# LaurenYTaylor/jsrl-CORL

Hardware: NVIDIA B200
Metric: iql_gradient_steps_per_sec_summed_over_seeds (higher is better)
Workload: dtype tf32

## Files before the change

include/iql_b200.h:

```cpp
#ifndef IQL_B200_H
#define IQL_B200_H

#include <stddef.h>
#include <stdint.h>

#ifdef __cplusplus
extern "C" {
#endif

#define IQL_OK 0
#define IQL_ERR_INVALID 1
#define IQL_ERR_CUDA 2
#define IQL_ERR_STATE 3
#define IQL_ERR_SHAPE 4

#define IQL_MATH_FP32_SIMT 0
#define IQL_MATH_TF32_TCGEN05 1

#define IQL_SAMPLE_PHILOX 0
#define IQL_SAMPLE_INDICES 1
#define IQL_SAMPLE_PRELOADED 2

#define IQL_NET_Q1 0
#define IQL_NET_Q2 1
// ... 144 lines not shown
                         float* host_out, float* host_std, void* stream, void* caller_stream);
int iql_get_act_steps(iql_engine* e, uint64_t* host_out);
int iql_set_act_steps(iql_engine* e, const uint64_t* host_in);
int iql_replay_insert_members_host(iql_engine* e, const float* host_states, const float* host_actions,
                                   const float* host_rewards, const float* host_next_states, const float* host_dones,
                                   const int64_t* host_pointers, void* stream, void* caller_stream);
int iql_selftest_umma_gemm(int32_t mode, int32_t M, int32_t N, int32_t K, const float* A, int32_t lda,
                           const float* B, int32_t ldb, float* C, int32_t ldc, void* scratch,
                           size_t scratch_bytes, void* stream);
int iql_profile_step(iql_engine* e, int32_t reps, int32_t max_slots, int32_t* n_slots, float* avg_ms,
                     double* flops, double* bytes, char* labels, void* stream);
int64_t iql_last_launch_count(const iql_engine* e);
int iql_debug_fused_trace(long long* out, int32_t max_words);
int iql_debug_step_trace(iql_engine* e, int32_t reset, unsigned long long* out, int32_t max_words, void* stream);
int iql_debug_chain_trace(long long* out, int32_t max_words);

#ifdef __cplusplus
}
#endif
#endif
```

jsrl_corl_b200/_lib.py:

```python
from __future__ import annotations

import ctypes as C
import os

_HERE = os.path.dirname(os.path.abspath(__file__))
LIB_PATH = os.path.join(_HERE, "libiql_b200.so")
if os.environ.get("IQL_B200_DEBUG") and os.environ.get("IQL_B200_LIB"):
    LIB_PATH = os.environ["IQL_B200_LIB"]

IQL_OK, IQL_ERR_INVALID, IQL_ERR_CUDA, IQL_ERR_STATE, IQL_ERR_SHAPE = 0, 1, 2, 3, 4
MATH_FP32_SIMT, MATH_TF32_TCGEN05 = 0, 1
SAMPLE_PHILOX, SAMPLE_INDICES, SAMPLE_PRELOADED = 0, 1, 2
NET_Q1, NET_Q2, NET_V, NET_ACTOR = 0, 1, 2, 3
KIND_WEIGHT, KIND_BIAS, KIND_LOG_STD = 0, 1, 2
OPT_STEP_PATH, OPT_KEEP_GRADS = 1, 2
INFO_TENSOR_CORE_PATH, INFO_FUSED_FORWARD, INFO_CHAINED_BACKWARD, INFO_CHAINED_BACKWARD_GRADS = 1, 2, 3, 4
STEP_PATHS = {"auto": 0, "phases": 1, "chain": 2, "chain_grads": 4}
ACT_SKIP, ACT_LEARNER, ACT_LEARNER_DIST, ACT_GUIDE, ACT_LEARNER_DROPOUT, ACT_LEARNER_DIST_DROPOUT = 0, 1, 2, 3, 4, 5
ACT_SOURCES = {"skip": ACT_SKIP, "learner": ACT_LEARNER, "learner_dist": ACT_LEARNER_DIST, "guide": ACT_GUIDE,
               "learner_dropout": ACT_LEARNER_DROPOUT, "learner_dist_dropout": ACT_LEARNER_DIST_DROPOUT}


class Config(C.Structure):
    _fields_ = [
# ... 82 lines not shown
    "iql_load_batch": (C.c_int, [_P, C.c_int32, _P, _P, _P, _P, _P, _P]),
    "iql_train_steps": (C.c_int, [_P, C.c_int32, C.c_int32, _P, _P, _P, _P, _P]),
    "iql_train_host_step": (C.c_int, [_P, _P, _P, _P, _P]),
    "iql_host_step_wait": (C.c_int, [_P, _P, _P]),
    "iql_act": (C.c_int, [_P, C.c_int32, _P, C.c_int64, C.c_float, _P, _P]),
    "iql_act_host": (C.c_int, [_P, C.c_int32, _P, C.c_float, _P, _P, _P]),
    "iql_act_host_gaussian": (C.c_int, [_P, C.c_int32, _P, _P, _P, _P, _P]),
    "iql_bind_guide": (C.c_int, [_P, _P]),
    "iql_act_host_members": (C.c_int, [_P, _P, _P, C.c_float, _P, _P, _P, _P]),
    "iql_get_act_steps": (C.c_int, [_P, _P]),
    "iql_set_act_steps": (C.c_int, [_P, _P]),
    "iql_replay_insert_members_host": (C.c_int, [_P, _P, _P, _P, _P, _P, _P, _P, _P]),
    "iql_last_launch_count": (C.c_int64, [_P]),
    "iql_debug_fused_trace": (C.c_int, [_P, C.c_int32]),
    "iql_debug_chain_trace": (C.c_int, [_P, C.c_int32]),
    "iql_debug_step_trace": (C.c_int, [_P, C.c_int32, _P, C.c_int32, _P]),
    "iql_profile_step": (C.c_int, [_P, C.c_int32, C.c_int32, C.POINTER(C.c_int32), _P, _P, _P, _P, _P]),
    "iql_selftest_umma_gemm": (C.c_int, [C.c_int32, C.c_int32, C.c_int32, C.c_int32, _P, C.c_int32, _P, C.c_int32,
                                          _P, C.c_int32, _P, C.c_size_t, _P]),
}

_LIB = None


def lib() -> C.CDLL:
    global _LIB
    if _LIB is None:
        if not os.path.exists(LIB_PATH):
            raise RuntimeError(
                f"{LIB_PATH} is missing: the CUDA engine is the only compute path of jsrl_corl_b200 "
# ... 35 lines not shown
```

jsrl_corl_b200/csrc/common.cuh:

```cuda
#pragma once
#include <cuda_runtime.h>
#include <stdint.h>
#include <stdlib.h>
#include <string.h>

namespace iql {

#define IQL_PHILOX_M0 0xD2511F53u
#define IQL_PHILOX_M1 0xCD9E8D57u
#define IQL_PHILOX_W0 0x9E3779B9u
#define IQL_PHILOX_W1 0xBB67AE85u

#define IQL_STREAM_SAMPLE 0u
#define IQL_STREAM_DROPOUT_BASE 1u
#define IQL_STREAM_ACT_DROPOUT_BASE 0x80000000u

struct Philox4 {
  uint32_t x, y, z, w;
};

__host__ __device__ __forceinline__ void philox_mulhilo(uint32_t a, uint32_t b, uint32_t& hi, uint32_t& lo) {
  uint64_t p = (uint64_t)a * (uint64_t)b;
  hi = (uint32_t)(p >> 32);
  lo = (uint32_t)p;
// ... 48 lines not shown
  return (uint32_t)t;
}

__device__ __forceinline__ float round_tf32(float x) {
  return __uint_as_float((__float_as_uint(x) + 0x1000u) & 0xFFFFE000u);
}

static inline int64_t round_up(int64_t x, int64_t m) { return (x + m - 1) / m * m; }

static inline const char* dbg_getenv(const char* name) {
  static int on = -1;
  if (on < 0) on = getenv("IQL_B200_DEBUG") ? 1 : 0;
  return on ? getenv(name) : nullptr;
}

__device__ __forceinline__ void stamp_begin(unsigned long long* stamps, int slot) {
  if (stamps && threadIdx.x == 0) {
    unsigned long long t;
    asm volatile("mov.u64 %0, %%globaltimer;" : "=l"(t));
    atomicMin(stamps + 2 * slot, t);
  }
}
__device__ __forceinline__ void stamp_end(unsigned long long* stamps, int slot) {
  if (stamps && threadIdx.x == 0) {
    unsigned long long t;
    asm volatile("mov.u64 %0, %%globaltimer;" : "=l"(t));
    atomicMax(stamps + 2 * slot + 1, t);
  }
}

// ... 48 lines not shown
```

jsrl_corl_b200/csrc/engine.cu:

```cuda
#include <math.h>
#include <stdio.h>
#include <string.h>

#include <algorithm>
#include <atomic>
#include <chrono>
#include <map>
#include <tuple>
#include <string>
#include <type_traits>
#include <vector>

#include "common.cuh"
#include "engine.h"
#include "umma_gemm.h"

using namespace iql;

static thread_local std::string g_create_error;
static constexpr int CHAIN_GRADS_MIN_MEMBERS = 8;

struct StepTimer {
  std::vector<cudaEvent_t> ev;
  std::vector<std::string> label;
// ... 116 lines not shown
  std::vector<iql_counters> h_counters;
  std::vector<ReplayBinding> h_replay;
  std::vector<GemmProb> h_probs;
  std::vector<Phase> fwd_phases, bwd_phases;
  bool bound = false, tables_dirty = true, scalars_dirty = true, counters_dirty = true, replay_dirty = true;
  std::vector<char> preloaded;
  std::vector<int32_t> active;
  std::vector<char> is_active;
  int64_t last_launches = 0;
  std::string err;
  std::map<GraphKey, std::pair<cudaGraphExec_t, int64_t>> graphs;
  cudaStream_t side = nullptr;
  cudaEvent_t ev_fork = nullptr, ev_side = nullptr, ev_fork_g = nullptr, ev_gather = nullptr;
  bool use_graphs = true;
  unsigned long long* d_stamps = nullptr;
  float* h_act = nullptr;
  char* h_mail = nullptr;
  bool mail_pending = false;
  cudaStream_t host_step_stream = nullptr;
  bool host_step_stream_set = false;
  cudaEvent_t ev_in = nullptr;
  const float* guide = nullptr;
  char* h_actm = nullptr;
  std::vector<uint64_t> act_steps;
  char* h_ins = nullptr;
  int ins_slot = 0;
  int ins_n[2] = {0, 0};
  cudaStream_t ins_stream[2] = {nullptr, nullptr};
};

// ... 192 lines not shown

extern "C" void iql_destroy(iql_engine* e) {
  if (!e) return;
  drop_graphs(e);
  if (e->ev_fork) cudaEventDestroy(e->ev_fork);
  if (e->ev_side) cudaEventDestroy(e->ev_side);
  if (e->ev_fork_g) cudaEventDestroy(e->ev_fork_g);
  if (e->ev_gather) cudaEventDestroy(e->ev_gather);
  if (e->side) cudaStreamDestroy(e->side);
  if (e->ev_in) cudaEventDestroy(e->ev_in);
  if (e->h_mail) cudaFreeHost(e->h_mail);
  if (e->h_act) cudaFreeHost(e->h_act);
  if (e->h_actm) cudaFreeHost(e->h_actm);
  if (e->h_ins) cudaFreeHost(e->h_ins);
  if (e->d_stamps) cudaFree(e->d_stamps);
  delete e;
}

extern "C" int iql_get_layout(const iql_engine* e, iql_layout* out) {
  if (!e || !out) return IQL_ERR_INVALID;
  *out = e->layout;
  return IQL_OK;
}

extern "C" int iql_tensor_at(const iql_engine* e, int32_t index, iql_tensor_info* out) {
  if (!e || !out || index < 0 || index >= (int)e->tensors.size()) return IQL_ERR_INVALID;
  *out = e->tensors[index];
  return IQL_OK;
}

// ... 450 lines not shown
  e->ws = (char*)workspace; e->ws_bytes = workspace_bytes;
  place_tables(e, e->ws);
  e->d_ws_f = (float*)(e->ws + e->tables_bytes);
  int rc = bind_tables(e);
  if (rc != IQL_OK) return rc;
  if (!e->side) {
    if (cudaStreamCreateWithFlags(&e->side, cudaStreamNonBlocking) != cudaSuccess ||
        cudaEventCreateWithFlags(&e->ev_fork, cudaEventDisableTiming) != cudaSuccess ||
        cudaEventCreateWithFlags(&e->ev_side, cudaEventDisableTiming) != cudaSuccess ||
        cudaEventCreateWithFlags(&e->ev_fork_g, cudaEventDisableTiming) != cudaSuccess ||
        cudaEventCreateWithFlags(&e->ev_gather, cudaEventDisableTiming) != cudaSuccess) {
      cudaGetLastError();
      e->side = nullptr;
    }
  }
  if (dbg_getenv("IQL_STEP_TRACE") && !e->d_stamps && cudaMalloc((void**)&e->d_stamps, sizeof(unsigned long long) * 2 * ST_COUNT) != cudaSuccess) {
    cudaGetLastError();
    e->d_stamps = nullptr;
  }
  e->bound = true;
  e->tables_dirty = e->scalars_dirty = e->counters_dirty = e->replay_dirty = true;
  drop_graphs(e);
  return IQL_OK;
}

static int flush_tables(iql_engine* e, cudaStream_t st) {
  const int S = e->cfg.n_members, L = e->cfg.n_hidden;
  if (e->tables_dirty) {
    CUDA_TRY(e, cudaMemcpyAsync(e->d_probs, e->h_probs.data(), sizeof(GemmProb) * e->h_probs.size(), cudaMemcpyHostToDevice, st));
    CUDA_TRY(e, cudaMemcpyAsync(e->d_maps, e->h_maps.data(), e->h_maps.size(), cudaMemcpyHostToDevice, st));
// ... 2 lines not shown
    if (!e->h_maps_c.empty())
      CUDA_TRY(e, cudaMemcpyAsync(e->d_maps_c, e->h_maps_c.data(), e->h_maps_c.size(), cudaMemcpyHostToDevice, st));
    if (!e->h_maps_store.empty())
      CUDA_TRY(e, cudaMemcpyAsync(e->d_maps_store, e->h_maps_store.data(), e->h_maps_store.size(), cudaMemcpyHostToDevice, st));
    if (!e->h_maps_chain.empty())
      CUDA_TRY(e, cudaMemcpyAsync(e->d_maps_chain, e->h_maps_chain.data(), e->h_maps_chain.size(), cudaMemcpyHostToDevice, st));
    if (!e->h_maps_pol.empty())
      CUDA_TRY(e, cudaMemcpyAsync(e->d_maps_pol, e->h_maps_pol.data(), e->h_maps_pol.size(), cudaMemcpyHostToDevice, st));
    std::vector<int64_t> off(2 * (L + 1));
    for (int l = 0; l <= L; ++l) {
      off[l] = e->w_off[IQL_NET_ACTOR][l];
      off[L + 1 + l] = e->b_off[IQL_NET_ACTOR][l];
    }
    CUDA_TRY(e, cudaMemcpyAsync(e->d_act_off, off.data(), sizeof(int64_t) * off.size(), cudaMemcpyHostToDevice, st));
    CUDA_TRY(e, cudaMemcpyAsync(e->d_active, e->active.data(), sizeof(int32_t) * e->active.size(), cudaMemcpyHostToDevice, st));
    const size_t ring_row = sizeof(float) * 3 * (size_t)e->cfg.max_steps_per_call;
    for (int m = 0; m < S; ++m)
      if (!e->is_active[m]) CUDA_TRY(e, cudaMemsetAsync((char*)e->d_loss_ring + ring_row * m, 0xFF, ring_row, st));
    CUDA_TRY(e, cudaStreamSynchronize(st));
    e->tables_dirty = false;
  }
  if (e->scalars_dirty) {
    CUDA_TRY(e, cudaMemcpyAsync(e->d_scalars, e->h_scalars.data(), sizeof(MemberScalars) * S, cudaMemcpyHostToDevice, st));
    e->scalars_dirty = false;
  }
  if (e->counters_dirty) {
    CUDA_TRY(e, cudaMemcpyAsync(e->d_counters, e->h_counters.data(), sizeof(iql_counters) * S, cudaMemcpyHostToDevice, st));
    e->counters_dirty = false;
  }
  if (e->replay_dirty) {
// ... 33 lines not shown
  c.n_hid = 0;
  if (c.bias_hidden)
    for (int n = 0; n < 4; ++n)
      for (int l = 1; l < e->cfg.n_hidden; ++l) {
        c.hid_begin[c.n_hid] = e->w_off[n][l];
        c.hid_end[c.n_hid] = e->w_off[n][l] + (int64_t)e->cfg.hidden_dim * e->w_ld[n][l];
        ++c.n_hid;
      }
  const int Lh = e->cfg.n_hidden;
  c.first_w_begin[4] = e->pol_umma ? e->w_off[IQL_NET_ACTOR][Lh] : 0;
  c.first_w_end[4] = e->pol_umma ? e->w_off[IQL_NET_ACTOR][Lh] + (int64_t)e->cfg.action_dim * e->w_ld[IQL_NET_ACTOR][Lh] : 0;
  c.stamps = e->d_stamps;
  c.xrow_off_ = e->wl.xrow;
  c.xhi_off = (c.tf32 && e->split_first) ? e->wl.xhi : 0;
  c.xlo_off = (c.tf32 && e->split_first) ? e->wl.xlo : 0;
  return c;
}

extern "C" int iql_sync_target(iql_engine* e, int32_t member, void* stream) {
  if (!e || member < 0 || member >= e->cfg.n_members) return fail(e, IQL_ERR_INVALID, "iql_sync_target: bad member");
  if (!e->bound) return fail(e, IQL_ERR_STATE, "iql_sync_target: state not bound");
  const int64_t PQ = e->layout.q_floats, P = e->layout.param_floats;
  CUDA_TRY(e, cudaMemcpyAsync(e->target + member * PQ, e->params + member * P, PQ * sizeof(float), cudaMemcpyDeviceToDevice, (cudaStream_t)stream));
  return IQL_OK;
}

extern "C" int iql_bind_replay(iql_engine* e, int32_t member, const float* rows, int64_t capacity, int64_t size) {
  if (!e || member < 0 || member >= e->cfg.n_members) return fail(e, IQL_ERR_INVALID, "iql_bind_replay: bad member");
  if (!rows || capacity <= 0 || size < 0 || size > capacity) return fail(e, IQL_ERR_INVALID, "iql_bind_replay: bad rows/capacity/size");
  if ((uintptr_t)rows & 15) return fail(e, IQL_ERR_INVALID, "iql_bind_replay: rows must be 16-byte aligned");
// ... 61 lines not shown
    if (tm) tm->mark("gather", 0, 2.0 * S_d * e->cfg.batch_size * e->layout.row.row_floats * 4);
    launch_gather(ctx, e->d_ws_f, e->wl.member_floats, e->wl.xrow, st);
    ++launches;
  }
  const iql_config& c = e->cfg;
  const int B = c.batch_size, H = c.hidden_dim, A = c.action_dim, K0 = c.state_dim + c.action_dim;
  const bool first_ok = first_fwd_skinny_ok(K0);
  const bool first_wgrad_ok = first_wgrad_skinny_ok(B, K0);
  const bool out_ok = out_fwd_skinny_ok(H, A);
  const bool last_ok = last_bwd_skinny_ok(B, A);
  static const bool no_side = dbg_getenv("IQL_B200_NO_SIDE_STREAM") != nullptr;
  const bool loss_recomputed = last_ok && e->bwd_phases.size() >= 2 &&
                               last_bwd_recomputes_loss_grads(H, A, e->bwd_phases[0].count * e->lb_splits, B / e->lb_splits) &&
                               e->bwd_phases[0].kind == PH_LAST_WGRAD && e->bwd_phases[1].kind == PH_LAST_DGRAD &&
                               e->bwd_phases[0].count % 4 == 0;
  bool skip_next = false, skip_colsum = false;
  const bool lb_side = tf32_math && !tm && !no_side && e->side != nullptr;
  bool lb_on_side = false;
  auto run_phase = [&](const Phase& ph, const Phase* next, const Phase* next2) {
    if (skip_next) { skip_next = false; return; }
    const GemmProb* pp = e->d_probs + ph.first;
    const bool split = ph.kind == PH_FIRST_FWD && e->split_first;
    const bool umma = tf32_math && ph.umma_ok && umma_phase_supported(ph.mode, B, H) &&
                      !(ph.kind == PH_FIRST_FWD && !split && first_ok);
    const bool fuse_out = umma && ph.mode == 0 && ph.epi == EPI_RELU && next && next->kind == PH_OUT_FWD && H == 256 &&
                          umma_can_fuse_out(A);
    if (tm) {
      double fl = 0, by = 0;
      auto add = [&](const Phase& q) {
        for (int i = 0; i < q.count; ++i) {
// ... 478 lines not shown
  if (!e || !e->d_stamps) return -1;
  if (reset) {
    std::vector<unsigned long long> init(2 * ST_COUNT);
    for (int i = 0; i < ST_COUNT; ++i) { init[2 * i] = ~0ull; init[2 * i + 1] = 0ull; }
    if (cudaMemcpyAsync(e->d_stamps, init.data(), sizeof(unsigned long long) * init.size(), cudaMemcpyHostToDevice, (cudaStream_t)stream) != cudaSuccess ||
        cudaStreamSynchronize((cudaStream_t)stream) != cudaSuccess)
      return -2;
    return 0;
  }
  if (!out || max_words < 2 * ST_COUNT) return -1;
  if (cudaDeviceSynchronize() != cudaSuccess) return -2;
  if (cudaMemcpy(out, e->d_stamps, sizeof(unsigned long long) * 2 * ST_COUNT, cudaMemcpyDeviceToHost) != cudaSuccess) return -2;
  return 2 * ST_COUNT;
}

extern "C" int64_t iql_last_launch_count(const iql_engine* e) { return e ? e->last_launches : 0; }

extern "C" int iql_act(iql_engine* e, int32_t member, const float* states, int64_t n, float max_action,
                       float* out_actions, void* stream) {
  if (!e || member < -1 || member >= e->cfg.n_members) return fail(e, IQL_ERR_INVALID, "iql_act: bad member");
  if (!e->bound) return fail(e, IQL_ERR_STATE, "iql_act: state not bound");
  if (!states || !out_actions || n < 0) return fail(e, IQL_ERR_INVALID, "iql_act: null or negative n");
  if (n == 0) return IQL_OK;
  int rc = flush_tables(e, (cudaStream_t)stream);
  if (rc != IQL_OK) return rc;
  StepCtx ctx = make_ctx(e);
  const int L = e->cfg.n_hidden;
  const int first = member < 0 ? 0 : member, count = member < 0 ? e->cfg.n_members : 1;
  launch_act(ctx, e->params + (int64_t)first * e->layout.param_floats, count, e->d_act_off, e->d_act_off + (L + 1), states,
             n, max_action, out_actions, (cudaStream_t)stream);
// ... 288 lines not shown
```

jsrl_corl_b200/csrc/engine.h:

```cpp
#pragma once
#include <cuda_runtime.h>
#include <stdint.h>

#include <string>
#include <vector>

#include "../../include/iql_b200.h"

namespace iql {

int make_row_layout(int S, int A, iql_row_layout* out);

enum Epilogue : int {
  EPI_NONE = 0,
  EPI_LINEAR = 1,
  EPI_RELU = 2,
  EPI_DRELU = 3,
};

struct GemmProb {
  const float* A;
  const float* B;
  float* C;
  const float* bias;
// ... 61 lines not shown
  unsigned long long* stamps;
  AdamScalars* adam_sc;
  int k_max;
  int tf32;
  float* w_shadow;
  float* t_shadow;
  float* w_shadow_lo;
  float* t_shadow_lo;
  int64_t first_w_begin[5], first_w_end[5];
  int bias_hidden;
  int unbias_out;
  int n_hid;
  int64_t hid_begin[4 * 3], hid_end[4 * 3];
  int64_t xrow_off_;
  int64_t xhi_off, xlo_off;
};

struct TensorDesc {
  iql_tensor_info info;
};

struct WorkspaceLayout {
  int64_t xrow;
  int64_t act;
  int64_t yq;
  int64_t zpi;
  int64_t gy;
  int64_t gpi;
  int64_t gh;
  int64_t xhi, xlo;
// ... 13 lines not shown
                      const StepCtx& ctx, cudaStream_t st);
void launch_gather(const StepCtx& ctx, float* ws, int64_t ws_member_floats, int64_t xrow_off, cudaStream_t st);
void launch_loss(const StepCtx& ctx, float* ws, int64_t ws_member_floats, const WorkspaceLayout& wl,
                 const float* params, float* grads, cudaStream_t st);
void launch_adam(const StepCtx& ctx, float* params, float* exp_avg, float* exp_avg_sq, float* target,
                 const float* grads, cudaStream_t st);
void launch_advance(const StepCtx& ctx, int K, cudaStream_t st);
void launch_refresh_shadow(const StepCtx& ctx, float* params, float* target, cudaStream_t st);
void launch_gather_refresh(const StepCtx& ctx, float* ws, int64_t ws_member_floats, int64_t xrow_off, float* params, float* target,
                           cudaStream_t st);
void launch_load_batch(const StepCtx& ctx, int member, float* xrow, const float* s, const float* a, const float* r,
                       const float* s2, const float* d, cudaStream_t st);
void launch_first_fwd(const GemmProb* probs, int nprob, int B, int H, int kmax, const StepCtx& ctx, cudaStream_t st);
void launch_out_fwd(const GemmProb* probs, int nprob, int B, int H, int amax, cudaStream_t st);
bool last_bwd_recomputes_loss_grads(int H, int amax, int nprob, int B);
void launch_lb_reduce(const GemmProb* pw_split, const GemmProb* prev_split, const GemmProb* pw, const GemmProb* prev, int nprob,
                      int splits, cudaStream_t st);
int launch_last_bwd(const GemmProb* probs_dgrad, const GemmProb* probs_wgrad, const GemmProb* probs_prev_wgrad,
                     int nprob, int B, int H, int amax, const StepCtx& ctx, cudaStream_t st, const float* ws = nullptr,
                     int64_t ws_member_floats = 0, const WorkspaceLayout* wl = nullptr, const float* params = nullptr);
void launch_first_wgrad(const GemmProb* probs, int nprob, int B, int H, int kmax, cudaStream_t st);
void launch_act(const StepCtx& ctx, const float* actor_block, int n_members, const int64_t* w_off,
                const int64_t* b_off, const float* states, int64_t n, float max_action, float* out, cudaStream_t st);

int act_host_state_max();
void launch_act_host(const StepCtx& ctx, const float* actor_block, const int64_t* w_off, const int64_t* b_off,
                     const float* host_state, float max_action, const float* log_std , float* mail,
                     cudaStream_t st);
void launch_act_members(const StepCtx& ctx, const float* params, const float* guide, const int64_t* w_off, const int64_t* b_off,
                        const float* states, const int32_t* ids, const int32_t* codes, const uint64_t* steps, bool drop_codes,
// ... 6 lines not shown
```

jsrl_corl_b200/csrc/fused_fwd.cu:

```cuda
#include <cuda.h>
#include <stdio.h>
#include <stdlib.h>
#include <string.h>

#include "common.cuh"
#include "tcgen05.cuh"
#include "umma_gemm.h"

namespace iql {

namespace {

constexpr int FT_M = 128, FT_N = 256, FT_K = 32, F_UMMA_K = 8;
constexpr int F_STAGE_A = FT_M * FT_K * 4;
constexpr int F_STAGE_B = FT_N * FT_K * 4;
constexpr int F_STAGE = F_STAGE_A + F_STAGE_B;
constexpr int F_STAGES = 3;
constexpr int F_GRAN = 16 * 1024, F_NGRAN = 9, F_MAXBAR = 9;
constexpr int F_NA = 4, F_NB = F_NGRAN - F_NA;
constexpr int F_EPI_WARPS = 16, F_EGROUPS = 2, F_GROUP_WARPS = F_EPI_WARPS / F_EGROUPS, F_CGROUPS = 2, F_CHUNKS = FT_N / 32;
constexpr int F_STG_FLOATS = 32 * 32;
constexpr int F_RING = F_STAGES * F_STAGE;
constexpr int F_STG_BYTES = F_EPI_WARPS * F_STG_FLOATS * 4;
constexpr int F_REC_FLOATS = FUSED_MAX_LAYERS * FT_N + FT_N + 64;
// ... 100 lines not shown
  const uint32_t tmem_base = *tslot_ptr;
  life_stamp(1);
  pdl_wait();
  life_stamp(2);
  const int nkb_h = FT_N / FT_K;
  const uint32_t rank = CTA2 ? cluster_ctarank() : 0u;
  const int worker = CTA2 ? (int)(blockIdx.x >> 1) : (int)blockIdx.x;
  const int n_workers = CTA2 ? (int)(gridDim.x >> 1) : (int)gridDim.x;
  const int tile_rows = CTA2 ? 2 * FT_M : FT_M;
  const int m_off = (int)rank * FT_M;

  if (warp == 0) {
    if (lane == 0) {
      uint32_t stage = 0, phase = 0, bphase = 0, tile_it = 0;
      for (int u = worker; u < fp.units; u += n_workers, ++tile_it) {
        const int prob = unit_prob(fp, u);
        const int m0 = (u % fp.tiles_m) * tile_rows + m_off;
        {
          const int un = u + n_workers;
          if (un < fp.units) {
            const int pn = unit_prob(fp, un);
            if (pn != prob) {
              for (int i = 0; i < 4; ++i) asm volatile("prefetch.tensormap [%0];" ::"l"(fp.maps[0] + 4 * pn + i) : "memory");
              for (int l = 1; l < L; ++l) asm volatile("prefetch.tensormap [%0];" ::"l"(fp.maps[l] + 2 * pn + 1) : "memory");
              for (int l = 0; l < L; ++l) asm volatile("prefetch.tensormap [%0];" ::"l"(fp.smaps[l] + pn) : "memory");
            }
          }
        }
        if (CTA2) {
          const uint32_t full_lead = mapa_u32(full0, 0);
// ... 220 lines not shown
    }
  } else {
    const int q = warp & 3;
    const int eg = (warp - 2) / F_GROUP_WARPS;
    const int ch = ((warp - 2) % F_GROUP_WARPS) >> 2;
    const bool wide = fp.wide != 0;
    const int cg = wide ? eg * F_CGROUPS + ch : ch;
    const int n_cg = wide ? F_EGROUPS * F_CGROUPS : F_CGROUPS;
    const int tr_id = wide ? (int)threadIdx.x - 64 : (int)threadIdx.x - 64 - eg * (F_GROUP_WARPS * 32);
    const int bar_id = wide ? 3 : 1 + eg, bar_n = wide ? F_EPI_WARPS * 32 : F_GROUP_WARPS * 32;
    const bool tracer = ((warp - 2) % F_GROUP_WARPS) == 0 && lane == 0 && (!wide || eg == 0);
    float* stg = stg_all + (warp - 2) * F_STG_FLOATS;
    uint32_t ev = 0, tile_it = 0;
    const uint32_t elast_lead = CTA2 ? mapa_u32(elast, 0) : elast;
    const uint32_t achunk_lead = CTA2 ? mapa_u32(achunk0, 0) : achunk0;
    for (int u = worker; u < fp.units; u += n_workers, ++tile_it) {
      if (!wide && (int)(tile_it & 1) != eg) continue;
      const int prob = unit_prob(fp, u);
      const int m0 = (u % fp.tiles_m) * tile_rows + m_off;
      const uint32_t b = tile_it & 1;
      const float* rec = rec_s + b * F_REC_FLOATS;
      ev = (tile_it >> 1) * (uint32_t)L;
      mbar_wait(recfull0 + 8 * b, (tile_it >> 1) & 1);
      const TileRec* tr = reinterpret_cast<const TileRec*>(rec + FUSED_MAX_LAYERS * FT_N + FT_N);
      const bool store = tr->store != 0;
      const int row = m0 + q * 32 + lane;
      for (int l = 0; l < L; ++l, ++ev) {
        const bool last = (l == L - 1);
        const bool fuse = last && tr->fuse;
        const int drop_layer = tr->drop_layer[l];
        const uint32_t drop_thr = (drop_layer >= 0) ? tr->drop_thr : 0u;
        const bool drop = drop_thr != 0u;
// ... 164 lines not shown
#pragma unroll
                for (int g4 = 0; g4 < F_EGROUPS * F_CGROUPS; ++g4)
                  if (g4 < n_cg) z += p0[g4 * 4 * F_STG_FLOATS];
                zrow[a] = z + tr->pol_b[a];
              }
            }
          }
          asm volatile("bar.sync %0, %1;" ::"r"(bar_id), "r"(bar_n) : "memory");
        }
        if (tracer) trace_put(fp, 2, tile_it, l, 3);
      }
      __syncwarp();
      if (lane == 0 && !wide) mbar_arrive(recempty0 + 8 * b);
    }
    bulk_wait0();
  }
  tc_fence_before();
  __syncwarp();
  if (CTA2) cluster_sync();
  else __syncthreads();
  if (warp == 1) {
    if (CTA2) asm volatile("tcgen05.dealloc.cta_group::2.sync.aligned.b32 %0, %1;" ::"r"(tmem_base), "r"(512u) : "memory");
    else asm volatile("tcgen05.dealloc.cta_group::1.sync.aligned.b32 %0, %1;" ::"r"(tmem_base), "r"(512u) : "memory");
  }
  life_stamp(3);
  stamp_end(ctx.stamps, ST_FWD);
}

}

// ... 88 lines not shown
```

jsrl_corl_b200/csrc/kernels_skinny.cu:

```cuda
#include <stdlib.h>
#include <string.h>

#include <algorithm>

#include "common.cuh"
#include "engine.h"

namespace iql {

template <int KMAX, int NC>
__global__ void __launch_bounds__(128) first_fwd_kernel(const GemmProb* __restrict__ probs, StepCtx ctx) {
  constexpr int RT = 64;
  __shared__ __align__(16) float xs[RT][KMAX];
  const GemmProb p = probs[blockIdx.x];
  const int r0 = blockIdx.y * RT;
  const int nb = blockIdx.z * 128 * NC + threadIdx.x;
  const int K = p.K;
  if (r0 >= p.M) return;
  for (int i = threadIdx.x; i < RT * KMAX; i += 128) {
    const int r = i / KMAX, k = i - r * KMAX;
    float v = 0.f;
    if (r0 + r < p.M && k < K) v = p.A[(int64_t)(r0 + r) * p.lda + k];
    xs[r][k] = v;
  }
// ... 281 lines not shown
        const float s = ((red[(0 * 64 + tn) * AMAX + m] + red[(1 * 64 + tn) * AMAX + m]) +
                         red[(2 * 64 + tn) * AMAX + m]) + red[(3 * 64 + tn) * AMAX + m];
        pw.C[(int64_t)m * pw.ldc + n] = s;
      }
    }
    if (dbias_prev != nullptr) dbias_prev[n] = ((cred[0][tn] + cred[1][tn]) + cred[2][tn]) + cred[3][tn];
  }
  if (blockIdx.y == 0 && pw.dbias != nullptr && threadIdx.x < AO) {
    float s = 0.f;
    for (int b = 0; b < B; ++b) s += gs[b * AMAX + threadIdx.x];
    pw.dbias[threadIdx.x] = s;
  }
}

template <int AMAX>
__device__ __forceinline__ void loss_row_grads(const StepCtx& ctx, const MemberScalars& sc, const float* __restrict__ w,
                                               const WorkspaceLayout& wl, const float* __restrict__ log_std, int t, int b,
                                               float* g) {
  const int B = ctx.B, RF = ctx.row.row_floats;
#pragma unroll
  for (int a = 0; a < AMAX; ++a) g[a] = 0.f;
  if (b >= sc.batch) return;
  const float* yq = w + wl.yq;
  const float inv_b = 1.0f / (float)sc.batch;
  const float v = yq[PASS_V * B + b];
  const float tq = fminf(yq[PASS_TQ1 * B + b], yq[PASS_TQ2 * B + b]);
  const float adv = tq - v;
  if (t == 0) {
    const float w_neg = fabsf(sc.iql_tau - 1.0f), w_pos = fabsf(sc.iql_tau);
    const float wt = adv < 0.f ? w_neg : w_pos;
    g[0] = -((wt * inv_b) * (2.0f * adv));
// ... 25 lines not shown
          const float sd = expf(ls);
          const float var = sd * sd;
          const float diff = act - mu;
          gmu = -eb * diff / var;
        }
        g[a] = gmu * (1.0f - mu * mu);
      }
    }
  }
}

template <int AMAX>
__global__ void __launch_bounds__(256) last_bwd_v4_kernel(const GemmProb* __restrict__ probs_dgrad,
                                                          const GemmProb* __restrict__ probs_wgrad,
                                                          const GemmProb* __restrict__ probs_prev_wgrad, StepCtx ctx,
                                                          const float* __restrict__ ws, int64_t ws_member_floats,
                                                          WorkspaceLayout wl, const float* __restrict__ params, int sel_n,
                                                          int sel_off) {
  extern __shared__ float sm[];
  stamp_begin(ctx.stamps, ST_LASTBWD);
  pdl_trigger();
  const int pi = sel_n > 0 ? (int)(blockIdx.x / sel_n) * 4 + sel_off + (int)(blockIdx.x % sel_n) : (int)blockIdx.x;
  const GemmProb pn = probs_dgrad[pi];
  const GemmProb pw = probs_wgrad[pi];
  float* dbias_prev = probs_prev_wgrad ? probs_prev_wgrad[pi].dbias : nullptr;
  pdl_wait();
  const int B = pn.M, H = pn.N, AO = pn.K;
  float* gs = sm;
  float* red = sm + (size_t)B * AMAX;
  if (ws != nullptr) {
    const MemberScalars msc = ctx.scalars[pn.member];
    const float* wmem = ws + (int64_t)pn.member * ws_member_floats;
    const float* log_std = params + (int64_t)pn.member * ctx.P + ctx.log_std_off;
    const int t = pi & 3;
    for (int b = threadIdx.x; b < B; b += 256) {
      float g[AMAX];
      loss_row_grads<AMAX>(ctx, msc, wmem, wl, log_std, t, b + pn.row0, g);
#pragma unroll
      for (int a = 0; a < AMAX; ++a) gs[b * AMAX + a] = g[a];
    }
  } else {
// ... 12 lines not shown
    dw[m] = make_float4(0.f, 0.f, 0.f, 0.f);
  }
  const MemberScalars* sc = ctx.scalars + pn.member;
  const float dscale = (pn.drop_layer >= 0 && sc->drop_threshold != 0u) ? sc->drop_scale : 1.0f;
  const bool tf32 = ctx.tf32 != 0;
  __syncthreads();
  const int rows_per = (B + 3) / 4;
  const int b_lo = bg * rows_per, b_hi = min(B, b_lo + rows_per);
  float4 csum = make_float4(0.f, 0.f, 0.f, 0.f);
  if (act) {
    constexpr int RB = 8;
    for (int b0 = b_lo; b0 < b_hi; b0 += RB) {
      float4 hv[RB];
#pragma unroll
      for (int j = 0; j < RB; ++j)
        hv[j] = (b0 + j < b_hi) ? __ldg(reinterpret_cast<const float4*>(pn.mask + (int64_t)(b0 + j) * pn.ldmask + n))
                                : make_float4(0.f, 0.f, 0.f, 0.f);
#pragma unroll
      for (int j = 0; j < RB; ++j) {
        if (b0 + j < b_hi) {
          float4 gsum = make_float4(0.f, 0.f, 0.f, 0.f);
          if (AO == 1) {
            const float g = gs[(b0 + j) * AMAX];
            gsum.x = g * w[0].x; gsum.y = g * w[0].y; gsum.z = g * w[0].z; gsum.w = g * w[0].w;
            dw[0].x = fmaf(g, hv[j].x, dw[0].x); dw[0].y = fmaf(g, hv[j].y, dw[0].y);
            dw[0].z = fmaf(g, hv[j].z, dw[0].z); dw[0].w = fmaf(g, hv[j].w, dw[0].w);
          } else {
#pragma unroll
            for (int m = 0; m < AMAX; ++m) {
              const float g = gs[(b0 + j) * AMAX + m];
              gsum.x = fmaf(g, w[m].x, gsum.x); gsum.y = fmaf(g, w[m].y, gsum.y);
// ... 29 lines not shown
#pragma unroll
    for (int g = 0; g < 4; ++g) s += red[(g * 256 + col) * RS + m];
    if (m < AO) pw.C[(int64_t)m * pw.ldc + nn] = s;
    else if (m == AMAX && dbias_prev != nullptr) dbias_prev[nn] = s;
  }
  if (blockIdx.y == 0 && pw.dbias != nullptr && threadIdx.x < AO) {
    float s = 0.f;
    for (int b = 0; b < B; ++b) s += gs[b * AMAX + threadIdx.x];
    pw.dbias[threadIdx.x] = s;
  }
  stamp_end(ctx.stamps, ST_LASTBWD);
}

static bool last_bwd_v4_fills(int nprob, int B, int H) { return !(B >= 2048 && (int64_t)nprob * ((H + 255) / 256) < 64); }

bool last_bwd_recomputes_loss_grads(int H, int amax, int nprob, int B) {
  return dbg_getenv("IQL_B200_NO_LASTBWD_V4") == nullptr && dbg_getenv("IQL_B200_NO_LOSS_OVERLAP") == nullptr && (H % 4) == 0 && amax <= 8 &&
         last_bwd_v4_fills(nprob, B, H);
}

int launch_last_bwd(const GemmProb* probs_dgrad, const GemmProb* probs_wgrad, const GemmProb* probs_prev_wgrad,
                     int nprob, int B, int H, int amax, const StepCtx& ctx, cudaStream_t st, const float* ws,
                     int64_t ws_member_floats, const WorkspaceLayout* wl, const float* params) {
  dim3 grid(nprob, (H + 63) / 64);
  auto smem = [&](int a) { return ((size_t)B * a + 4 * 64 * a) * sizeof(float); };
  auto smem4 = [&](int a) { return ((size_t)B * a + 4 * 256 * (a + 1)) * sizeof(float); };
  static bool attr[64] = {};
  static bool no_v4 = false;
  if (first_use_on_device(attr)) {
    cudaFuncSetAttribute(last_bwd_kernel<24>, cudaFuncAttributeMaxDynamicSharedMemorySize, 200 * 1024);
    cudaFuncSetAttribute(last_bwd_kernel<8>, cudaFuncAttributeMaxDynamicSharedMemorySize, 200 * 1024);
    cudaFuncSetAttribute(last_bwd_kernel<1>, cudaFuncAttributeMaxDynamicSharedMemorySize, 200 * 1024);
    cudaFuncSetAttribute(last_bwd_v4_kernel<8>, cudaFuncAttributeMaxDynamicSharedMemorySize, 200 * 1024);
    cudaFuncSetAttribute(last_bwd_v4_kernel<1>, cudaFuncAttributeMaxDynamicSharedMemorySize, 200 * 1024);
    no_v4 = dbg_getenv("IQL_B200_NO_LASTBWD_V4") != nullptr;
  }
  const bool v4 = !no_v4 && (H % 4) == 0 && amax <= 8 && smem4(8) <= 200 * 1024 && last_bwd_v4_fills(nprob, B, H);
  const dim3 grid4(nprob, (H + 255) / 256);
  WorkspaceLayout wlv;
  memset(&wlv, 0, sizeof(wlv));
  if (wl) wlv = *wl;
  const float* wsp = (wl && nprob % 4 == 0) ? ws : nullptr;
  if (v4 && amax <= 1)
    launch_pdl(last_bwd_v4_kernel<1>, grid4, dim3(256), smem4(1), st, 1, probs_dgrad, probs_wgrad, probs_prev_wgrad, ctx, wsp,
               ws_member_floats, wlv, params, 0, 0);
  else if (v4)
    launch_pdl(last_bwd_v4_kernel<8>, grid4, dim3(256), smem4(8), st, 1, probs_dgrad, probs_wgrad, probs_prev_wgrad, ctx, wsp,
               ws_member_floats, wlv, params, 0, 0);
  else if (amax <= 1) last_bwd_kernel<1><<<grid, 256, smem(1), st>>>(probs_dgrad, probs_wgrad, probs_prev_wgrad, ctx, 0, 0);
  else if (amax <= 8) last_bwd_kernel<8><<<grid, 256, smem(8), st>>>(probs_dgrad, probs_wgrad, probs_prev_wgrad, ctx, 0, 0);
  else if (!no_v4 && (H % 4) == 0 && nprob % 4 == 0 && wl != nullptr && smem4(1) <= 200 * 1024) {
    launch_pdl(last_bwd_v4_kernel<1>, dim3(nprob / 4 * 3, (H + 255) / 256), dim3(256), smem4(1), st, 1, probs_dgrad, probs_wgrad,
// ... 136 lines not shown
```

Baseline: 220,300.

## Hand off fused forward tiles to last-layer backward via per-member ready counters

Adds per-member global ready counters that the fused forward kernel's epilogue increments (release semantics) after each tile's results are stored. The last-layer backward v4 kernel now spins on its member's counter instead of waiting on the whole preceding grid through PDL. The forward kernel also triggers PDL early, on its last tile, so the backward can launch and start as soon as its member's forward work is done. This overlaps the tail of the forward with the start of the backward, at the cost of spin-waiting, counter reset logic, and a switch from __ldg to __ldcg and a dropped __restrict__ so data written concurrently is read coherently.

```diff
diff --git a/include/iql_b200.h b/include/iql_b200.h
--- a/include/iql_b200.h
+++ b/include/iql_b200.h
@@ -182,6 +182,7 @@
 int iql_debug_fused_trace(long long* out, int32_t max_words);
 int iql_debug_step_trace(iql_engine* e, int32_t reset, unsigned long long* out, int32_t max_words, void* stream);
 int iql_debug_chain_trace(long long* out, int32_t max_words);
+int iql_debug_fwd_ready(iql_engine* e, uint32_t* out, int32_t max_words);
 
 #ifdef __cplusplus
 }
diff --git a/jsrl_corl_b200/_lib.py b/jsrl_corl_b200/_lib.py
--- a/jsrl_corl_b200/_lib.py
+++ b/jsrl_corl_b200/_lib.py
@@ -120,6 +120,7 @@
     "iql_last_launch_count": (C.c_int64, [_P]),
     "iql_debug_fused_trace": (C.c_int, [_P, C.c_int32]),
     "iql_debug_chain_trace": (C.c_int, [_P, C.c_int32]),
+    "iql_debug_fwd_ready": (C.c_int, [_P, _P, C.c_int32]),
     "iql_debug_step_trace": (C.c_int, [_P, C.c_int32, _P, C.c_int32, _P]),
     "iql_profile_step": (C.c_int, [_P, C.c_int32, C.c_int32, C.POINTER(C.c_int32), _P, _P, _P, _P, _P]),
     "iql_selftest_umma_gemm": (C.c_int, [C.c_int32, C.c_int32, C.c_int32, C.c_int32, _P, C.c_int32, _P, C.c_int32,
diff --git a/jsrl_corl_b200/csrc/common.cuh b/jsrl_corl_b200/csrc/common.cuh
--- a/jsrl_corl_b200/csrc/common.cuh
+++ b/jsrl_corl_b200/csrc/common.cuh
@@ -86,6 +86,19 @@
   return on ? getenv(name) : nullptr;
 }
 
+__device__ __forceinline__ void ready_wait(const uint32_t* c, uint32_t n) {
+  for (uint32_t spins = 0;; ++spins) {
+    uint32_t v;
+    asm volatile("ld.acquire.gpu.global.u32 %0, [%1];" : "=r"(v) : "l"(c) : "memory");
+    if (v >= n) return;
+    if (spins > (1u << 24)) __trap();
+    __nanosleep(64);
+  }
+}
+__device__ __forceinline__ void ready_publish(uint32_t* c) {
+  __threadfence();
+  asm volatile("red.release.gpu.global.add.u32 [%0], 1;" ::"l"(c) : "memory");
+}
 __device__ __forceinline__ void stamp_begin(unsigned long long* stamps, int slot) {
   if (stamps && threadIdx.x == 0) {
     unsigned long long t;
diff --git a/jsrl_corl_b200/csrc/engine.cu b/jsrl_corl_b200/csrc/engine.cu
--- a/jsrl_corl_b200/csrc/engine.cu
+++ b/jsrl_corl_b200/csrc/engine.cu
@@ -154,6 +154,7 @@
   cudaEvent_t ev_fork = nullptr, ev_side = nullptr, ev_fork_g = nullptr, ev_gather = nullptr;
   bool use_graphs = true;
   unsigned long long* d_stamps = nullptr;
+  uint32_t* d_fwd_ready = nullptr;
   float* h_act = nullptr;
   char* h_mail = nullptr;
   bool mail_pending = false;
@@ -376,6 +377,7 @@
   if (e->h_actm) cudaFreeHost(e->h_actm);
   if (e->h_ins) cudaFreeHost(e->h_ins);
   if (e->d_stamps) cudaFree(e->d_stamps);
+  if (e->d_fwd_ready) cudaFree(e->d_fwd_ready);
   delete e;
 }
 
@@ -856,6 +858,10 @@
       e->side = nullptr;
     }
   }
+  if (!e->d_fwd_ready && cudaMalloc((void**)&e->d_fwd_ready, sizeof(uint32_t) * e->cfg.n_members) != cudaSuccess) {
+    e->d_fwd_ready = nullptr;
+    CUDA_TRY(e, cudaGetLastError());
+  }
   if (dbg_getenv("IQL_STEP_TRACE") && !e->d_stamps && cudaMalloc((void**)&e->d_stamps, sizeof(unsigned long long) * 2 * ST_COUNT) != cudaSuccess) {
     cudaGetLastError();
     e->d_stamps = nullptr;
@@ -888,6 +894,7 @@
     }
     CUDA_TRY(e, cudaMemcpyAsync(e->d_act_off, off.data(), sizeof(int64_t) * off.size(), cudaMemcpyHostToDevice, st));
     CUDA_TRY(e, cudaMemcpyAsync(e->d_active, e->active.data(), sizeof(int32_t) * e->active.size(), cudaMemcpyHostToDevice, st));
+    CUDA_TRY(e, cudaMemsetAsync(e->d_fwd_ready, 0, sizeof(uint32_t) * S, st));
     const size_t ring_row = sizeof(float) * 3 * (size_t)e->cfg.max_steps_per_call;
     for (int m = 0; m < S; ++m)
       if (!e->is_active[m]) CUDA_TRY(e, cudaMemsetAsync((char*)e->d_loss_ring + ring_row * m, 0xFF, ring_row, st));
@@ -951,6 +958,7 @@
   c.xrow_off_ = e->wl.xrow;
   c.xhi_off = (c.tf32 && e->split_first) ? e->wl.xhi : 0;
   c.xlo_off = (c.tf32 && e->split_first) ? e->wl.xlo : 0;
+  c.fwd_ready = e->d_fwd_ready;
   return c;
 }
 
@@ -1042,6 +1050,12 @@
                                last_bwd_recomputes_loss_grads(H, A, e->bwd_phases[0].count * e->lb_splits, B / e->lb_splits) &&
                                e->bwd_phases[0].kind == PH_LAST_WGRAD && e->bwd_phases[1].kind == PH_LAST_DGRAD &&
                                e->bwd_phases[0].count % 4 == 0;
+  {
+    const bool handoff = tf32_math && e->fused_fwd && fused_fwd_policy_head(A) && loss_recomputed && e->lb_splits == 1 &&
+                         last_bwd_v4_single(e->bwd_phases[0].count, B, H, A);
+    const int ctas = e->fused_pair ? 2 : 1, tile_rows = 128 * ctas;
+    ctx.fwd_ready_n = handoff ? (uint32_t)(e->fwd_phases[0].count / (int)e->active.size() * ((B + tile_rows - 1) / tile_rows) * ctas) : 0u;
+  }
   bool skip_next = false, skip_colsum = false;
   const bool lb_side = tf32_math && !tm && !no_side && e->side != nullptr;
   bool lb_on_side = false;
@@ -1550,6 +1564,14 @@
   return 2 * ST_COUNT;
 }
 
+extern "C" int iql_debug_fwd_ready(iql_engine* e, uint32_t* out, int32_t max_words) {
+  const int n = e ? e->cfg.n_members : 0;
+  if (!e || !e->d_fwd_ready || !out || max_words < n) return -1;
+  if (cudaDeviceSynchronize() != cudaSuccess) return -2;
+  if (cudaMemcpy(out, e->d_fwd_ready, sizeof(uint32_t) * n, cudaMemcpyDeviceToHost) != cudaSuccess) return -2;
+  return n;
+}
+
 extern "C" int64_t iql_last_launch_count(const iql_engine* e) { return e ? e->last_launches : 0; }
 
 extern "C" int iql_act(iql_engine* e, int32_t member, const float* states, int64_t n, float max_action,
diff --git a/jsrl_corl_b200/csrc/engine.h b/jsrl_corl_b200/csrc/engine.h
--- a/jsrl_corl_b200/csrc/engine.h
+++ b/jsrl_corl_b200/csrc/engine.h
@@ -99,6 +99,8 @@
   int64_t hid_begin[4 * 3], hid_end[4 * 3];
   int64_t xrow_off_;
   int64_t xhi_off, xlo_off;
+  uint32_t* fwd_ready;
+  uint32_t fwd_ready_n;
 };
 
 struct TensorDesc {
@@ -142,6 +144,7 @@
 void launch_first_fwd(const GemmProb* probs, int nprob, int B, int H, int kmax, const StepCtx& ctx, cudaStream_t st);
 void launch_out_fwd(const GemmProb* probs, int nprob, int B, int H, int amax, cudaStream_t st);
 bool last_bwd_recomputes_loss_grads(int H, int amax, int nprob, int B);
+bool last_bwd_v4_single(int nprob, int B, int H, int amax);
 void launch_lb_reduce(const GemmProb* pw_split, const GemmProb* prev_split, const GemmProb* pw, const GemmProb* prev, int nprob,
                       int splits, cudaStream_t st);
 int launch_last_bwd(const GemmProb* probs_dgrad, const GemmProb* probs_wgrad, const GemmProb* probs_prev_wgrad,
diff --git a/jsrl_corl_b200/csrc/fused_fwd.cu b/jsrl_corl_b200/csrc/fused_fwd.cu
--- a/jsrl_corl_b200/csrc/fused_fwd.cu
+++ b/jsrl_corl_b200/csrc/fused_fwd.cu
@@ -138,6 +138,7 @@
     if (lane == 0) {
       uint32_t stage = 0, phase = 0, bphase = 0, tile_it = 0;
       for (int u = worker; u < fp.units; u += n_workers, ++tile_it) {
+        if (ctx.fwd_ready_n && fp.units > n_workers && u + n_workers >= fp.units) pdl_trigger();
         const int prob = unit_prob(fp, u);
         const int m0 = (u % fp.tiles_m) * tile_rows + m_off;
         {
@@ -388,8 +389,17 @@
     uint32_t ev = 0, tile_it = 0;
     const uint32_t elast_lead = CTA2 ? mapa_u32(elast, 0) : elast;
     const uint32_t achunk_lead = CTA2 ? mapa_u32(achunk0, 0) : achunk0;
+    auto publish = [&](int uu) {
+      if (lane == 0) {
+        bulk_wait0();
+        asm volatile("fence.proxy.async;" ::: "memory");
+      }
+      asm volatile("bar.sync %0, %1;" ::"r"(bar_id), "r"(bar_n) : "memory");
+      if (tr_id == 0) ready_publish(ctx.fwd_ready + fp.probs[0][unit_prob(fp, uu)].member);
+    };
     for (int u = worker; u < fp.units; u += n_workers, ++tile_it) {
       if (!wide && (int)(tile_it & 1) != eg) continue;
+      if (ctx.fwd_ready_n && tile_it >= 2) publish(u - 2 * n_workers);
       const int prob = unit_prob(fp, u);
       const int m0 = (u % fp.tiles_m) * tile_rows + m_off;
       const uint32_t b = tile_it & 1;
@@ -584,6 +594,11 @@
       if (lane == 0 && !wide) mbar_arrive(recempty0 + 8 * b);
     }
     bulk_wait0();
+    if (ctx.fwd_ready_n) {
+      const int n_tiles = (fp.units - worker + n_workers - 1) / n_workers;
+      const int t_last = wide ? 0 : ((((n_tiles - 1) & 1) == eg) ? n_tiles - 1 : n_tiles - 2);
+      if (t_last >= 0) publish(worker + t_last * n_workers);
+    }
   }
   tc_fence_before();
   __syncwarp();
diff --git a/jsrl_corl_b200/csrc/kernels_skinny.cu b/jsrl_corl_b200/csrc/kernels_skinny.cu
--- a/jsrl_corl_b200/csrc/kernels_skinny.cu
+++ b/jsrl_corl_b200/csrc/kernels_skinny.cu
@@ -319,7 +319,7 @@
 }
 
 template <int AMAX>
-__device__ __forceinline__ void loss_row_grads(const StepCtx& ctx, const MemberScalars& sc, const float* __restrict__ w,
+__device__ __forceinline__ void loss_row_grads(const StepCtx& ctx, const MemberScalars& sc, const float* w,
                                                const WorkspaceLayout& wl, const float* __restrict__ log_std, int t, int b,
                                                float* g) {
   const int B = ctx.B, RF = ctx.row.row_floats;
@@ -375,17 +375,28 @@
 __global__ void __launch_bounds__(256) last_bwd_v4_kernel(const GemmProb* __restrict__ probs_dgrad,
                                                           const GemmProb* __restrict__ probs_wgrad,
                                                           const GemmProb* __restrict__ probs_prev_wgrad, StepCtx ctx,
-                                                          const float* __restrict__ ws, int64_t ws_member_floats,
+                                                          const float* ws, int64_t ws_member_floats,
                                                           WorkspaceLayout wl, const float* __restrict__ params, int sel_n,
                                                           int sel_off) {
   extern __shared__ float sm[];
   stamp_begin(ctx.stamps, ST_LASTBWD);
-  pdl_trigger();
+  if (!ctx.fwd_ready_n) pdl_trigger();
   const int pi = sel_n > 0 ? (int)(blockIdx.x / sel_n) * 4 + sel_off + (int)(blockIdx.x % sel_n) : (int)blockIdx.x;
   const GemmProb pn = probs_dgrad[pi];
   const GemmProb pw = probs_wgrad[pi];
   float* dbias_prev = probs_prev_wgrad ? probs_prev_wgrad[pi].dbias : nullptr;
-  pdl_wait();
+  if (ctx.fwd_ready_n) {
+    if (threadIdx.x == 0) {
+      uint32_t* c = ctx.fwd_ready + pn.member;
+      ready_wait(c, ctx.fwd_ready_n);
+      const uint32_t blocks = gridDim.x / (uint32_t)ctx.n_active * gridDim.y;
+      if (atomicAdd(c, 1u) == ctx.fwd_ready_n + blocks - 1) atomicExch(c, 0u);
+    }
+    __syncthreads();
+    pdl_trigger();
+  } else {
+    pdl_wait();
+  }
   const int B = pn.M, H = pn.N, AO = pn.K;
   float* gs = sm;
   float* red = sm + (size_t)B * AMAX;
@@ -428,7 +439,7 @@
       float4 hv[RB];
 #pragma unroll
       for (int j = 0; j < RB; ++j)
-        hv[j] = (b0 + j < b_hi) ? __ldg(reinterpret_cast<const float4*>(pn.mask + (int64_t)(b0 + j) * pn.ldmask + n))
+        hv[j] = (b0 + j < b_hi) ? __ldcg(reinterpret_cast<const float4*>(pn.mask + (int64_t)(b0 + j) * pn.ldmask + n))
                                 : make_float4(0.f, 0.f, 0.f, 0.f);
 #pragma unroll
       for (int j = 0; j < RB; ++j) {
@@ -488,6 +499,11 @@
 
 static bool last_bwd_v4_fills(int nprob, int B, int H) { return !(B >= 2048 && (int64_t)nprob * ((H + 255) / 256) < 64); }
 
+bool last_bwd_v4_single(int nprob, int B, int H, int amax) {
+  return dbg_getenv("IQL_B200_NO_LASTBWD_V4") == nullptr && (H % 4) == 0 && amax <= 8 &&
+         ((size_t)B * 8 + 4 * 256 * 9) * sizeof(float) <= 200 * 1024 && last_bwd_v4_fills(nprob, B, H);
+}
+
 bool last_bwd_recomputes_loss_grads(int H, int amax, int nprob, int B) {
   return dbg_getenv("IQL_B200_NO_LASTBWD_V4") == nullptr && dbg_getenv("IQL_B200_NO_LOSS_OVERLAP") == nullptr && (H % 4) == 0 && amax <= 8 &&
          last_bwd_v4_fills(nprob, B, H);
@@ -509,7 +525,7 @@
     cudaFuncSetAttribute(last_bwd_v4_kernel<1>, cudaFuncAttributeMaxDynamicSharedMemorySize, 200 * 1024);
     no_v4 = dbg_getenv("IQL_B200_NO_LASTBWD_V4") != nullptr;
   }
-  const bool v4 = !no_v4 && (H % 4) == 0 && amax <= 8 && smem4(8) <= 200 * 1024 && last_bwd_v4_fills(nprob, B, H);
+  const bool v4 = last_bwd_v4_single(nprob, B, H, amax);
   const dim3 grid4(nprob, (H + 255) / 256);
   WorkspaceLayout wlv;
   memset(&wlv, 0, sizeof(wlv));
```

Result: slower. 215,600, median of 6 (-2.1%).
